# Neuroprosthetics-Lab/nejm-brain-to-text

Hardware: AMD Instinct MI355X
Metric: GRU+CTC train sentences/sec (higher is better)
Workload: dtype f32; 1 GPU; BASELINE.json configs[1]: 5-layer GRU-512 + CTC, synthetic [B=64,T=500,F=512] -> 41 phonemes, fp32, full training step incl. on-GPU augmentation, clip and AdamW; global_batch=64, rows_per_rank=64, seq_len=500, parallelism=dp1, world_size_seen=1, gru_mode=1

## Files before the change

nejm-brain-to-text_amd/csrc/gemm.hip:

```cpp
#include "common.h"
#include "gemm_args.h"

namespace b2t {

using f32x16 = float __attribute__((ext_vector_type(16)));
using f32x4 = float __attribute__((ext_vector_type(4)));

#ifndef B2T_GEMM_BK
#define B2T_GEMM_BK 16
#endif
#ifndef B2T_GEMM_OCC
#define B2T_GEMM_OCC 3
#endif
constexpr int BM = 128, BN = 128, BKT = B2T_GEMM_BK;
constexpr int NLD = BKT / 8;
constexpr int TPR = BKT / 4;
constexpr int RPP = 256 / TPR;
template <bool KC> struct Pitch { static constexpr int v = KC ? 129 : 132; };
constexpr int PITCH_MAX = 132;

template <bool KC>
__device__ __forceinline__ void load_full(const float* __restrict__ P, const long long (&roff)[NLD], int mcl, int k0,
                                          long long s0, long long s1, int div, float4 (&v)[NLD], int tid) {
#pragma unroll
  for (int r = 0; r < NLD; ++r) {
    if constexpr (KC) {
      v[r] = *reinterpret_cast<const float4*>(P + roff[r] + k0 + (tid % TPR) * 4);
    } else {
      v[r] = *reinterpret_cast<const float4*>(P + rowoff(k0 + (tid >> 5) + 8 * r, s0, s1, div) + mcl);
    }
  }
}

template <bool KC>
__device__ __forceinline__ void load_tail(const float* __restrict__ P, const long long (&roff)[NLD], int ext_m,
                                          int base_m, int k0, int Kend, long long s0, long long s1, int div,
                                          float4 (&v)[NLD], int tid) {
#pragma unroll
  for (int r = 0; r < NLD; ++r) {
    float4 o = make_float4(0.f, 0.f, 0.f, 0.f);
    if constexpr (KC) {
      const int row = base_m + tid / TPR + RPP * r;
      const int k = k0 + (tid % TPR) * 4;
      if (row < ext_m) {
        const float* p = P + roff[r] + k;
        if (k < Kend) o.x = p[0];
        if (k + 1 < Kend) o.y = p[1];
        if (k + 2 < Kend) o.z = p[2];
        if (k + 3 < Kend) o.w = p[3];
      }
    } else {
      const int k = k0 + (tid >> 5) + 8 * r;
      const int m = base_m + (tid & 31) * 4;
      if (k < Kend) {
        const float* p = P + rowoff(k, s0, s1, div) + m;
        if (m < ext_m) o.x = p[0];
        if (m + 1 < ext_m) o.y = p[1];
        if (m + 2 < ext_m) o.z = p[2];
        if (m + 3 < ext_m) o.w = p[3];
      }
    }
    v[r] = o;
  }
}

template <bool KC>
__device__ __forceinline__ void store_tile(float* __restrict__ S, const float4 (&v)[NLD], int tid) {
  constexpr int PITCH = Pitch<KC>::v;
#pragma unroll
  for (int r = 0; r < NLD; ++r) {
    if constexpr (KC) {
      const int row = tid / TPR + RPP * r;
      const int k = (tid % TPR) * 4;
      S[(k + 0) * PITCH + row] = v[r].x;
      S[(k + 1) * PITCH + row] = v[r].y;
      S[(k + 2) * PITCH + row] = v[r].z;
      S[(k + 3) * PITCH + row] = v[r].w;
    } else {
      const int k = (tid >> 5) + 8 * r;
      const int m = (tid & 31) * 4;
      *reinterpret_cast<float4*>(&S[k * PITCH + m]) = v[r];
    }
  }
}

__device__ __forceinline__ float4 load_f4_sc1(const float* base_uniform, unsigned byte_off) {
  using u32x4 = unsigned int __attribute__((ext_vector_type(4)));
  __amdgpu_buffer_rsrc_t rsrc = __builtin_amdgcn_make_buffer_rsrc(const_cast<float*>(base_uniform), 0, 0x7fffffff, 0x00020000);
  const u32x4 v = __builtin_amdgcn_raw_buffer_load_b128(rsrc, byte_off, 0, 16);
  return make_float4(__uint_as_float(v.x), __uint_as_float(v.y), __uint_as_float(v.z), __uint_as_float(v.w));
}

template <bool AKC, bool BKC>
__global__ __launch_bounds__(256, B2T_GEMM_OCC) void gemm_f32_kernel(GemmArgs g) {
  __shared__ __attribute__((aligned(16))) float smem[2 * 2 * BKT * PITCH_MAX];
  constexpr int PA = Pitch<AKC>::v, PB = Pitch<BKC>::v;
  float* As = smem;
  float* Bs = smem + 2 * BKT * PITCH_MAX;

  const int tid = threadIdx.x;
  const int lane = tid & 63, wave = tid >> 6;
  const int wm = wave >> 1, wn = wave & 1;
  int z = blockIdx.z / g.splitk;
  int ks = blockIdx.z - z * g.splitk;
  int m0, n0;
  {
    const int gx = (g.N + BN - 1) / BN, nwg = gridDim.x;
    int tile;
    if (g.ks_xcd) {
      const int lin = blockIdx.x + nwg * blockIdx.z, xcd = lin & 7, j = lin >> 3;
      ks = xcd + 8 * (j / nwg); tile = j % nwg; z = 0;
    } else {
      const int b = blockIdx.x, xcd = b & 7, qq = nwg >> 3, rr = nwg & 7;
      tile = (xcd < rr ? xcd * (qq + 1) : rr * (qq + 1) + (xcd - rr) * qq) + (b >> 3);
    }
    m0 = (tile / gx) * BM; n0 = (tile % gx) * BN;
  }

  const float* A = g.A + (long long)z * g.a_sz;
  const int zb = g.b_zmap ? g.b_zmap[z] : z;
  const float* B = g.B + (long long)zb * g.b_sz;
  const float* bias = (g.bias && ks == 0) ? g.bias + (long long)zb * g.bias_sz : nullptr;
  float* C = g.C + (long long)z * g.c_sz + (long long)ks * g.c_ks;

  long long roffA[NLD], roffB[NLD];
#pragma unroll
  for (int r = 0; r < NLD; ++r) {
    const int ra_ = m0 + tid / TPR + RPP * r, rb_ = n0 + tid / TPR + RPP * r;
    roffA[r] = AKC ? rowoff(ra_ < g.M ? ra_ : g.M - 1, g.a_s0, g.a_s1, g.a_div) : 0;
    roffB[r] = BKC ? rowoff(rb_ < g.N ? rb_ : g.N - 1, g.b_s0, g.b_s1, g.b_div) : 0;
  }
  const int mclA = min(m0 + (tid & 31) * 4, ((g.M + 3) & ~3) - 4);
  const int mclB = min(n0 + (tid & 31) * 4, ((g.N + 3) & ~3) - 4);

  f32x16 acc[2][2];
#pragma unroll
  for (int i = 0; i < 2; ++i)
#pragma unroll
    for (int j = 0; j < 2; ++j)
#pragma unroll
      for (int e = 0; e < 16; ++e) acc[i][j][e] = 0.f;

  const int kb = ks * g.kchunk;
  const int K = min(g.K, kb + g.kchunk);
  const int nk = (K - kb + BKT - 1) / BKT;
  const int nfull = (K - kb) / BKT;
  float4 ra[NLD], rb[NLD];

  auto fetch = [&](int kt) {
    const int k0 = kb + kt * BKT;
    const float* Ag = A + ((g.a_brk > 0 && (AKC ? k0 : m0) >= g.a_brk) ? g.a_gap : 0);
    if (kt < nfull) {
      load_full<AKC>(Ag, roffA, mclA, k0, g.a_s0, g.a_s1, g.a_div, ra, tid);
      load_full<BKC>(B, roffB, mclB, k0, g.b_s0, g.b_s1, g.b_div, rb, tid);
    } else {
      load_tail<AKC>(Ag, roffA, g.M, m0, k0, K, g.a_s0, g.a_s1, g.a_div, ra, tid);
      load_tail<BKC>(B, roffB, g.N, n0, k0, K, g.b_s0, g.b_s1, g.b_div, rb, tid);
    }
  };
  const bool do_sum = !AKC && g.a_sum != nullptr && n0 == 0;
  float4 asum = make_float4(0.f, 0.f, 0.f, 0.f);
  auto add_a = [&]() {
    if constexpr (!AKC) {
      if (do_sum) {
#pragma unroll
        for (int r = 0; r < NLD; ++r) { asum.x += ra[r].x; asum.y += ra[r].y; asum.z += ra[r].z; asum.w += ra[r].w; }
      }
    }
  };
  fetch(0);
  add_a();
  store_tile<AKC>(As, ra, tid);
  store_tile<BKC>(Bs, rb, tid);
  __syncthreads();

  const int lk = lane >> 5, li = lane & 31;
  int cur = 0;
  for (int kt = 0; kt < nk; ++kt) {
    const bool more = kt + 1 < nk;
    if (more) fetch(kt + 1);
    const float* as = As + cur * BKT * PA + wm * 64 + li + lk * PA;
    const float* bs = Bs + cur * BKT * PB + wn * 64 + li + lk * PB;
    float a0 = as[0], a1 = as[32], b0 = bs[0], b1 = bs[32];
#pragma unroll
    for (int kk = 0; kk < BKT; kk += 2) {
      float na0 = 0.f, na1 = 0.f, nb0 = 0.f, nb1 = 0.f;
      if (kk + 2 < BKT) {
        na0 = as[(kk + 2) * PA]; na1 = as[(kk + 2) * PA + 32];
        nb0 = bs[(kk + 2) * PB]; nb1 = bs[(kk + 2) * PB + 32];
      }
      acc[0][0] = __builtin_amdgcn_mfma_f32_32x32x2f32(a0, b0, acc[0][0], 0, 0, 0);
      acc[0][1] = __builtin_amdgcn_mfma_f32_32x32x2f32(a0, b1, acc[0][1], 0, 0, 0);
      acc[1][0] = __builtin_amdgcn_mfma_f32_32x32x2f32(a1, b0, acc[1][0], 0, 0, 0);
      acc[1][1] = __builtin_amdgcn_mfma_f32_32x32x2f32(a1, b1, acc[1][1], 0, 0, 0);
      a0 = na0; a1 = na1; b0 = nb0; b1 = nb1;
    }
    if (more) {
      add_a();
      store_tile<AKC>(As + (cur ^ 1) * BKT * PA, ra, tid);
      store_tile<BKC>(Bs + (cur ^ 1) * BKT * PB, rb, tid);
    }
    __syncthreads();
    cur ^= 1;
  }

  if constexpr (!AKC) {
    if (do_sum) {
      float4* red = reinterpret_cast<float4*>(smem);
      red[tid] = asum;
      __syncthreads();
      if (tid < 32) {
        float4 t = red[tid];
#pragma unroll
        for (int gq = 1; gq < 8; ++gq) { const float4 u = red[gq * 32 + tid]; t.x += u.x; t.y += u.y; t.z += u.z; t.w += u.w; }
        float* o = g.a_sum + ((long long)z * g.splitk + ks) * g.a_sum_ks;
        const int m = m0 + tid * 4;
        if (m < g.M) o[m] = t.x;
        if (m + 1 < g.M) o[m + 1] = t.y;
        if (m + 2 < g.M) o[m + 2] = t.z;
        if (m + 3 < g.M) o[m + 3] = t.w;
      }
    }
  }
#pragma unroll
  for (int i = 0; i < 2; ++i) {
#pragma unroll
    for (int j = 0; j < 2; ++j) {
      const int col = n0 + wn * 64 + j * 32 + li;
      if (col >= g.N) continue;
      const float bv = bias ? bias[col] : 0.f;
#pragma unroll
      for (int e = 0; e < 16; ++e) {
        const int row = m0 + wm * 64 + i * 32 + (e & 3) + 8 * (e >> 2) + 4 * lk;
        if (row < g.M) {
          float v = acc[i][j][e] + bv;
          if (g.epilogue == 1) v = v / (1.0f + fabsf(v));
          const long long coff = rowoff(row, g.c_s0, g.c_s1, g.c_div) + col;
          if (g.epilogue == 2) { const float a = 1.0f - fabsf(g.ep_aux[(long long)z * g.c_sz + coff]); v *= a * a; }
          float* p = C + coff;
          if (g.accumulate) v += *p;
          if (g.ks_cnt) __hip_atomic_store(p, v, __ATOMIC_RELAXED, __HIP_MEMORY_SCOPE_AGENT);
          else *p = v;
        }
      }
    }
  }
  if (g.ks_cnt) {
    asm volatile("s_waitcnt vmcnt(0)" ::: "memory");
    __syncthreads();
    int* flag = reinterpret_cast<int*>(smem);
    const int gx = (g.N + BN - 1) / BN, tile_id = (m0 / BM) * gx + n0 / BN;
    if (tid == 0) {
      const unsigned old = __hip_atomic_fetch_add(g.ks_cnt + tile_id, 1u, __ATOMIC_RELAXED, __HIP_MEMORY_SCOPE_AGENT);
      const int last = old == (unsigned)g.splitk - 1u;
      if (last) __hip_atomic_store(g.ks_cnt + tile_id, 0u, __ATOMIC_RELAXED, __HIP_MEMORY_SCOPE_AGENT);
      flag[0] = last;
    }
    __syncthreads();
    if (flag[0]) {
      for (int idx = tid; idx < BM * (BN / 4); idx += 256) {
        const int r = m0 + idx / (BN / 4), cc = n0 + (idx % (BN / 4)) * 4;
        if (r >= g.M || cc >= g.N) continue;
        const long long e = (long long)r * g.N + cc;
        float4 acc = make_float4(0.f, 0.f, 0.f, 0.f);
        if (g.ks_acc) acc = *reinterpret_cast<const float4*>(g.ks_out + e);
        for (int sl = 0; sl < g.splitk; ++sl) {
          const float4 v = load_f4_sc1(g.C + (long long)sl * g.c_ks, (unsigned)(e * 4));
          acc.x += v.x; acc.y += v.y; acc.z += v.z; acc.w += v.w;
        }
        *reinterpret_cast<float4*>(g.ks_out + e) = acc;
      }
    }
  }
}


template <int MT, bool BKC>
__global__ __launch_bounds__(512) void gemm_skinny_kernel(GemmArgs g) {
  __shared__ float red[8][MT][4][64];
  const int tid = threadIdx.x, lane = tid & 63, wave = tid >> 6;
  const int j = lane & 15, q = lane >> 4;
  const int n0 = blockIdx.x * 16;
  const int z = blockIdx.y, zb = g.b_zmap ? g.b_zmap[z] : z;
  g.A += (long long)z * g.a_sz; g.B += (long long)zb * g.b_sz; g.C += (long long)z * g.c_sz;
  if (g.bias) g.bias += (long long)zb * g.bias_sz;
  const int ncol = n0 + j < g.N ? n0 + j : g.N - 1;
  const float* brow = BKC ? g.B + rowoff(ncol, g.b_s0, g.b_s1, g.b_div) + 4 * q : g.B + ncol;
  const float* arow[MT];
#pragma unroll
  for (int mt = 0; mt < MT; ++mt) {
    const int r = 16 * mt + j;
    arow[mt] = g.A + rowoff(r < g.M ? r : g.M - 1, g.a_s0, g.a_s1, g.a_div) + 4 * q;
  }
  f32x4 acc[MT];
#pragma unroll
  for (int mt = 0; mt < MT; ++mt) acc[mt] = f32x4{0.f, 0.f, 0.f, 0.f};
  const int nchunk = g.K / 16;
  for (int c0 = wave * 4; c0 < nchunk; c0 += 32) {
    float4 bw[4], av[4][MT];
#pragma unroll
    for (int u = 0; u < 4; ++u) {
      const int k = (c0 + u < nchunk ? c0 + u : c0) * 16;
      if constexpr (BKC) {
        bw[u] = *reinterpret_cast<const float4*>(brow + k);
      } else {
        const int kq = k + 4 * q;
        bw[u] = make_float4(brow[rowoff(kq, g.b_s0, g.b_s1, g.b_div)], brow[rowoff(kq + 1, g.b_s0, g.b_s1, g.b_div)],
                            brow[rowoff(kq + 2, g.b_s0, g.b_s1, g.b_div)], brow[rowoff(kq + 3, g.b_s0, g.b_s1, g.b_div)]);
      }
#pragma unroll
      for (int mt = 0; mt < MT; ++mt) av[u][mt] = *reinterpret_cast<const float4*>(arow[mt] + k);
    }
#pragma unroll
    for (int u = 0; u < 4; ++u) {
      if (c0 + u < nchunk) {
#pragma unroll
        for (int mt = 0; mt < MT; ++mt) {
          acc[mt] = __builtin_amdgcn_mfma_f32_16x16x4f32(av[u][mt].x, bw[u].x, acc[mt], 0, 0, 0);
          acc[mt] = __builtin_amdgcn_mfma_f32_16x16x4f32(av[u][mt].y, bw[u].y, acc[mt], 0, 0, 0);
          acc[mt] = __builtin_amdgcn_mfma_f32_16x16x4f32(av[u][mt].z, bw[u].z, acc[mt], 0, 0, 0);
          acc[mt] = __builtin_amdgcn_mfma_f32_16x16x4f32(av[u][mt].w, bw[u].w, acc[mt], 0, 0, 0);
        }
      }
    }
  }
#pragma unroll
  for (int mt = 0; mt < MT; ++mt)
#pragma unroll
    for (int e = 0; e < 4; ++e) red[wave][mt][e][lane] = acc[mt][e];
  __syncthreads();
  for (int idx = tid; idx < MT * 4 * 64; idx += 512) {
    const int l = idx & 63, e = (idx >> 6) & 3, mt = idx >> 8;
    const float v0 = (red[0][mt][e][l] + red[1][mt][e][l]) + (red[2][mt][e][l] + red[3][mt][e][l]);
    const float v1 = (red[4][mt][e][l] + red[5][mt][e][l]) + (red[6][mt][e][l] + red[7][mt][e][l]);
    const int row = 16 * mt + 4 * (l >> 4) + e, col = n0 + (l & 15);
    if (row < g.M && col < g.N) {
      float v = v0 + v1 + (g.bias ? g.bias[col] : 0.f);
      if (g.epilogue == 1) v = v / (1.0f + fabsf(v));
      float* p = g.C + rowoff(row, g.c_s0, g.c_s1, g.c_div) + col;
      if (g.accumulate) v += *p;
      *p = v;
    }
  }
}

}

extern "C" int b2t_gemm_f32(const b2t_gemm_desc* d, void* stream) {
  using namespace b2t;
  B2T_REQUIRE(d != nullptr, "b2t_gemm_f32: null descriptor");
  B2T_REQUIRE(d->M > 0 && d->N > 0 && d->K > 0 && d->Z > 0, "b2t_gemm_f32: bad shape M=%d N=%d K=%d Z=%d",
              d->M, d->N, d->K, d->Z);
  B2T_REQUIRE(((uintptr_t)d->A & 15) == 0 && ((uintptr_t)d->B & 15) == 0, "b2t_gemm_f32: A/B must be 16-byte aligned");
  B2T_REQUIRE((d->a_s0 % 4) == 0 && (d->a_s1 % 4) == 0 && (d->a_sz % 4) == 0 && (d->b_s0 % 4) == 0 &&
                  (d->b_s1 % 4) == 0 && (d->b_sz % 4) == 0,
              "b2t_gemm_f32: A/B strides must be multiples of 4 elements");
  B2T_REQUIRE(d->a_sum == nullptr || !d->a_kcontig, "b2t_gemm_f32: a_sum goes with an m-contiguous A (a_kcontig = 0)");
  B2T_REQUIRE(d->ks_counters == nullptr || (d->splitk > 1 && d->Z == 1 && (d->N % 4) == 0 && d->ks_out != nullptr && ((uintptr_t)d->ks_out & 15) == 0 &&
                                            (long long)d->M * d->N * 4 < (1ll << 31)),
              "b2t_gemm_f32: the in-kernel slab reduction needs splitk > 1, Z = 1, N %% 4 == 0 and a 16-byte aligned ks_out");
  GemmArgs g;
  { int rc = fill_gemm_args(d, g, BKT, BM, "b2t_gemm_f32"); if (rc) return rc; }
  dim3 grid(((d->N + BN - 1) / BN) * ((d->M + BM - 1) / BM), 1, d->Z * g.splitk), block(256);
  { static const bool off = getenv("B2T_GEMM_KS_XCD") && atoi(getenv("B2T_GEMM_KS_XCD")) == 0; g.ks_xcd = !off && d->Z == 1 && g.splitk >= 8 && (g.splitk & 7) == 0; }
  hipStream_t s = as_stream(stream);
  if (d->M <= 64 && d->splitk >= 0 && g.splitk == 1 && d->a_kcontig && (d->K % 16) == 0 && d->a_brk == 0 && d->epilogue != 2) {
    const dim3 sg((d->N + 15) / 16, d->Z), sb(512);
#define B2T_SKINNY(MT)                                                                                  \
    do {                                                                                                \
      if (d->b_kcontig) hipLaunchKernelGGL((gemm_skinny_kernel<MT, true>), sg, sb, 0, s, g);              \
      else hipLaunchKernelGGL((gemm_skinny_kernel<MT, false>), sg, sb, 0, s, g);                          \
    } while (0)
    if (d->M <= 16) B2T_SKINNY(1);
    else if (d->M <= 32) B2T_SKINNY(2);
    else if (d->M <= 48) B2T_SKINNY(3);
    else B2T_SKINNY(4);
#undef B2T_SKINNY
    B2T_CHECK_LAUNCH("b2t_gemm_f32 (skinny)");
    return 0;
  }
  if (d->a_kcontig && d->b_kcontig) hipLaunchKernelGGL((gemm_f32_kernel<true, true>), grid, block, 0, s, g);
  else if (d->a_kcontig && !d->b_kcontig) hipLaunchKernelGGL((gemm_f32_kernel<true, false>), grid, block, 0, s, g);
  else if (!d->a_kcontig && d->b_kcontig) hipLaunchKernelGGL((gemm_f32_kernel<false, true>), grid, block, 0, s, g);
  else hipLaunchKernelGGL((gemm_f32_kernel<false, false>), grid, block, 0, s, g);
  B2T_CHECK_LAUNCH("b2t_gemm_f32");
  return 0;
}
```

Baseline: 3437 sentences/s.

## Use incremental address cursors and split main/tail loops in f32 GEMM

Replaces per-iteration rowoff index arithmetic with pointer cursors that advance by precomputed uniform strides, handling the div wrap and gap with selects. The k-loop is split into a steady full-tile loop without tail branching, separated by sched barriers, and a peeled tail. Launch bounds rise to occupancy 4 and the compile-time BK/OCC knobs are removed. This aims to cut VALU address work and register pressure in the GEMM main loop, at the cost of extra complexity and a possible correctness risk in the cursor wrap logic.

```diff
diff --git a/nejm-brain-to-text_amd/csrc/gemm.hip b/nejm-brain-to-text_amd/csrc/gemm.hip
--- a/nejm-brain-to-text_amd/csrc/gemm.hip
+++ b/nejm-brain-to-text_amd/csrc/gemm.hip
@@ -6,44 +6,84 @@
 using f32x16 = float __attribute__((ext_vector_type(16)));
 using f32x4 = float __attribute__((ext_vector_type(4)));
 
-#ifndef B2T_GEMM_BK
-#define B2T_GEMM_BK 16
-#endif
-#ifndef B2T_GEMM_OCC
-#define B2T_GEMM_OCC 3
-#endif
-constexpr int BM = 128, BN = 128, BKT = B2T_GEMM_BK;
+constexpr int BM = 128, BN = 128, BKT = 16;
 constexpr int NLD = BKT / 8;
 constexpr int TPR = BKT / 4;
 constexpr int RPP = 256 / TPR;
 template <bool KC> struct Pitch { static constexpr int v = KC ? 129 : 132; };
 constexpr int PITCH_MAX = 132;
 
+template <bool KC> struct Cursor {
+  const float* p[NLD];
+  int rem[NLD];
+  long long d0, d1;
+  int dv, stepr;
+};
+
+__device__ __forceinline__ int uniform(int v) { return __builtin_amdgcn_readfirstlane(v); }
+__device__ __forceinline__ long long uniform(long long v) {
+  return (long long)(((unsigned long long)(unsigned)uniform((int)(v >> 32)) << 32) | (unsigned)uniform((int)v));
+}
+
 template <bool KC>
-__device__ __forceinline__ void load_full(const float* __restrict__ P, const long long (&roff)[NLD], int mcl, int k0,
-                                          long long s0, long long s1, int div, float4 (&v)[NLD], int tid) {
+__device__ __forceinline__ void cursor_init(Cursor<KC>& c, const float* __restrict__ P, int base, int ext, int kb,
+                                            long long s0, long long s1, int div, int tid) {
+  if constexpr (KC) {
+#pragma unroll
+    for (int r = 0; r < NLD; ++r) {
+      const int row = base + tid / TPR + RPP * r;
+      c.p[r] = P + rowoff(row < ext ? row : ext - 1, s0, s1, div) + kb + (tid % TPR) * 4;
+      c.rem[r] = 0;
+    }
+    c.d0 = BKT; c.d1 = 0; c.dv = 0; c.stepr = 0;
+  } else {
+    c.dv = uniform(div > 0 ? div : 0x7fffffff);
+    c.stepr = uniform(BKT % c.dv);
+    c.d0 = uniform((long long)(BKT / c.dv) * s1 + (long long)c.stepr * s0);
+    c.d1 = uniform(s1 - (long long)c.dv * s0);
+    const int mcl = min(base + (tid & 31) * 4, ((ext + 3) & ~3) - 4);
+#pragma unroll
+    for (int r = 0; r < NLD; ++r) {
+      const int k = kb + (tid >> 5) + 8 * r;
+      c.rem[r] = k % c.dv;
+      c.p[r] = P + (long long)(k / c.dv) * s1 + (long long)c.rem[r] * s0 + mcl;
+    }
+  }
+}
+
+template <bool KC>
+__device__ __forceinline__ void cursor_next(Cursor<KC>& c, long long extra) {
 #pragma unroll
   for (int r = 0; r < NLD; ++r) {
     if constexpr (KC) {
-      v[r] = *reinterpret_cast<const float4*>(P + roff[r] + k0 + (tid % TPR) * 4);
+      c.p[r] += BKT + extra;
     } else {
-      v[r] = *reinterpret_cast<const float4*>(P + rowoff(k0 + (tid >> 5) + 8 * r, s0, s1, div) + mcl);
+      const int over = c.rem[r] + (c.stepr - c.dv);
+      const bool wrap = over >= 0;
+      c.rem[r] = wrap ? over : over + c.dv;
+      const float* same = c.p[r] + c.d0;
+      const float* wrapped = c.p[r] + (c.d0 + c.d1);
+      c.p[r] = wrap ? wrapped : same;
     }
   }
 }
 
 template <bool KC>
-__device__ __forceinline__ void load_tail(const float* __restrict__ P, const long long (&roff)[NLD], int ext_m,
-                                          int base_m, int k0, int Kend, long long s0, long long s1, int div,
-                                          float4 (&v)[NLD], int tid) {
+__device__ __forceinline__ void load_full(const Cursor<KC>& c, float4 (&v)[NLD]) {
+#pragma unroll
+  for (int r = 0; r < NLD; ++r) v[r] = *reinterpret_cast<const float4*>(c.p[r]);
+}
+
+template <bool KC>
+__device__ __forceinline__ void load_tail(const Cursor<KC>& c, int ext_m, int base_m, int k0, int Kend, float4 (&v)[NLD], int tid) {
 #pragma unroll
   for (int r = 0; r < NLD; ++r) {
     float4 o = make_float4(0.f, 0.f, 0.f, 0.f);
+    const float* p = c.p[r];
     if constexpr (KC) {
       const int row = base_m + tid / TPR + RPP * r;
       const int k = k0 + (tid % TPR) * 4;
       if (row < ext_m) {
-        const float* p = P + roff[r] + k;
         if (k < Kend) o.x = p[0];
         if (k + 1 < Kend) o.y = p[1];
         if (k + 2 < Kend) o.z = p[2];
@@ -53,7 +93,6 @@
       const int k = k0 + (tid >> 5) + 8 * r;
       const int m = base_m + (tid & 31) * 4;
       if (k < Kend) {
-        const float* p = P + rowoff(k, s0, s1, div) + m;
         if (m < ext_m) o.x = p[0];
         if (m + 1 < ext_m) o.y = p[1];
         if (m + 2 < ext_m) o.z = p[2];
@@ -84,6 +123,24 @@
   }
 }
 
+template <int PA, int PB>
+__device__ __forceinline__ void mma_tile(const float* __restrict__ as, const float* __restrict__ bs, f32x16 (&acc)[2][2]) {
+  float a0 = as[0], a1 = as[32], b0 = bs[0], b1 = bs[32];
+#pragma unroll
+  for (int kk = 0; kk < BKT; kk += 2) {
+    float na0 = 0.f, na1 = 0.f, nb0 = 0.f, nb1 = 0.f;
+    if (kk + 2 < BKT) {
+      na0 = as[(kk + 2) * PA]; na1 = as[(kk + 2) * PA + 32];
+      nb0 = bs[(kk + 2) * PB]; nb1 = bs[(kk + 2) * PB + 32];
+    }
+    acc[0][0] = __builtin_amdgcn_mfma_f32_32x32x2f32(a0, b0, acc[0][0], 0, 0, 0);
+    acc[0][1] = __builtin_amdgcn_mfma_f32_32x32x2f32(a0, b1, acc[0][1], 0, 0, 0);
+    acc[1][0] = __builtin_amdgcn_mfma_f32_32x32x2f32(a1, b0, acc[1][0], 0, 0, 0);
+    acc[1][1] = __builtin_amdgcn_mfma_f32_32x32x2f32(a1, b1, acc[1][1], 0, 0, 0);
+    a0 = na0; a1 = na1; b0 = nb0; b1 = nb1;
+  }
+}
+
 __device__ __forceinline__ float4 load_f4_sc1(const float* base_uniform, unsigned byte_off) {
   using u32x4 = unsigned int __attribute__((ext_vector_type(4)));
   __amdgpu_buffer_rsrc_t rsrc = __builtin_amdgcn_make_buffer_rsrc(const_cast<float*>(base_uniform), 0, 0x7fffffff, 0x00020000);
@@ -92,7 +149,7 @@
 }
 
 template <bool AKC, bool BKC>
-__global__ __launch_bounds__(256, B2T_GEMM_OCC) void gemm_f32_kernel(GemmArgs g) {
+__global__ __launch_bounds__(256, 4) void gemm_f32_kernel(GemmArgs g) {
   __shared__ __attribute__((aligned(16))) float smem[2 * 2 * BKT * PITCH_MAX];
   constexpr int PA = Pitch<AKC>::v, PB = Pitch<BKC>::v;
   float* As = smem;
@@ -123,16 +180,6 @@
   const float* bias = (g.bias && ks == 0) ? g.bias + (long long)zb * g.bias_sz : nullptr;
   float* C = g.C + (long long)z * g.c_sz + (long long)ks * g.c_ks;
 
-  long long roffA[NLD], roffB[NLD];
-#pragma unroll
-  for (int r = 0; r < NLD; ++r) {
-    const int ra_ = m0 + tid / TPR + RPP * r, rb_ = n0 + tid / TPR + RPP * r;
-    roffA[r] = AKC ? rowoff(ra_ < g.M ? ra_ : g.M - 1, g.a_s0, g.a_s1, g.a_div) : 0;
-    roffB[r] = BKC ? rowoff(rb_ < g.N ? rb_ : g.N - 1, g.b_s0, g.b_s1, g.b_div) : 0;
-  }
-  const int mclA = min(m0 + (tid & 31) * 4, ((g.M + 3) & ~3) - 4);
-  const int mclB = min(n0 + (tid & 31) * 4, ((g.N + 3) & ~3) - 4);
-
   f32x16 acc[2][2];
 #pragma unroll
   for (int i = 0; i < 2; ++i)
@@ -144,20 +191,16 @@
   const int kb = ks * g.kchunk;
   const int K = min(g.K, kb + g.kchunk);
   const int nk = (K - kb + BKT - 1) / BKT;
-  const int nfull = (K - kb) / BKT;
+  const int nfull = uniform(K > kb ? (K - kb) / BKT : 0);
+
+  const bool gap0 = g.a_brk > 0 && (AKC ? kb : m0) >= g.a_brk;
+  const int kgap = (AKC && g.a_brk > kb) ? g.a_brk : -1;
+  Cursor<AKC> ca;
+  Cursor<BKC> cb;
+  cursor_init<AKC>(ca, A + (gap0 ? g.a_gap : 0), m0, g.M, kb, g.a_s0, g.a_s1, g.a_div, tid);
+  cursor_init<BKC>(cb, B, n0, g.N, kb, g.b_s0, g.b_s1, g.b_div, tid);
   float4 ra[NLD], rb[NLD];
 
-  auto fetch = [&](int kt) {
-    const int k0 = kb + kt * BKT;
-    const float* Ag = A + ((g.a_brk > 0 && (AKC ? k0 : m0) >= g.a_brk) ? g.a_gap : 0);
-    if (kt < nfull) {
-      load_full<AKC>(Ag, roffA, mclA, k0, g.a_s0, g.a_s1, g.a_div, ra, tid);
-      load_full<BKC>(B, roffB, mclB, k0, g.b_s0, g.b_s1, g.b_div, rb, tid);
-    } else {
-      load_tail<AKC>(Ag, roffA, g.M, m0, k0, K, g.a_s0, g.a_s1, g.a_div, ra, tid);
-      load_tail<BKC>(B, roffB, g.N, n0, k0, K, g.b_s0, g.b_s1, g.b_div, rb, tid);
-    }
-  };
   const bool do_sum = !AKC && g.a_sum != nullptr && n0 == 0;
   float4 asum = make_float4(0.f, 0.f, 0.f, 0.f);
   auto add_a = [&]() {
@@ -168,53 +211,70 @@
       }
     }
   };
-  fetch(0);
+  auto next = [&](int k0) {
+    cursor_next<AKC>(ca, AKC && k0 == kgap ? g.a_gap : 0);
+    cursor_next<BKC>(cb, 0);
+  };
+  if (nfull > 0) {
+    load_full<AKC>(ca, ra);
+    load_full<BKC>(cb, rb);
+    next(kb + BKT);
+  } else {
+    load_tail<AKC>(ca, g.M, m0, kb, K, ra, tid);
+    load_tail<BKC>(cb, g.N, n0, kb, K, rb, tid);
+  }
   add_a();
   store_tile<AKC>(As, ra, tid);
   store_tile<BKC>(Bs, rb, tid);
   __syncthreads();
 
   const int lk = lane >> 5, li = lane & 31;
+  const float* as = As + wm * 64 + li + lk * PA;
+  const float* bs = Bs + wn * 64 + li + lk * PB;
   int cur = 0;
-  for (int kt = 0; kt < nk; ++kt) {
-    const bool more = kt + 1 < nk;
-    if (more) fetch(kt + 1);
-    const float* as = As + cur * BKT * PA + wm * 64 + li + lk * PA;
-    const float* bs = Bs + cur * BKT * PB + wn * 64 + li + lk * PB;
-    float a0 = as[0], a1 = as[32], b0 = bs[0], b1 = bs[32];
-#pragma unroll
-    for (int kk = 0; kk < BKT; kk += 2) {
-      float na0 = 0.f, na1 = 0.f, nb0 = 0.f, nb1 = 0.f;
-      if (kk + 2 < BKT) {
-        na0 = as[(kk + 2) * PA]; na1 = as[(kk + 2) * PA + 32];
-        nb0 = bs[(kk + 2) * PB]; nb1 = bs[(kk + 2) * PB + 32];
-      }
-      acc[0][0] = __builtin_amdgcn_mfma_f32_32x32x2f32(a0, b0, acc[0][0], 0, 0, 0);
-      acc[0][1] = __builtin_amdgcn_mfma_f32_32x32x2f32(a0, b1, acc[0][1], 0, 0, 0);
-      acc[1][0] = __builtin_amdgcn_mfma_f32_32x32x2f32(a1, b0, acc[1][0], 0, 0, 0);
-      acc[1][1] = __builtin_amdgcn_mfma_f32_32x32x2f32(a1, b1, acc[1][1], 0, 0, 0);
-      a0 = na0; a1 = na1; b0 = nb0; b1 = nb1;
-    }
-    if (more) {
-      add_a();
-      store_tile<AKC>(As + (cur ^ 1) * BKT * PA, ra, tid);
-      store_tile<BKC>(Bs + (cur ^ 1) * BKT * PB, rb, tid);
-    }
+#pragma unroll 1
+  for (int kt = 1; kt < nfull; ++kt) {
+    load_full<AKC>(ca, ra);
+    load_full<BKC>(cb, rb);
+    next(kb + (kt + 1) * BKT);
+    __builtin_amdgcn_sched_barrier(0);
+    mma_tile<PA, PB>(as + cur * BKT * PA, bs + cur * BKT * PB, acc);
+    __builtin_amdgcn_sched_barrier(0);
+    cur ^= 1;
+    add_a();
+    store_tile<AKC>(As + cur * BKT * PA, ra, tid);
+    store_tile<BKC>(Bs + cur * BKT * PB, rb, tid);
     __syncthreads();
+  }
+  int tp = tid;
+  asm volatile("" : "+v"(tp));
+  const bool tail = nfull > 0 && nk > nfull;
+  if (tail) {
+    load_tail<AKC>(ca, g.M, m0, kb + nfull * BKT, K, ra, tp);
+    load_tail<BKC>(cb, g.N, n0, kb + nfull * BKT, K, rb, tp);
+  }
+  if (nk > 0) mma_tile<PA, PB>(as + cur * BKT * PA, bs + cur * BKT * PB, acc);
+  if (tail) {
     cur ^= 1;
+    add_a();
+    store_tile<AKC>(As + cur * BKT * PA, ra, tp);
+    store_tile<BKC>(Bs + cur * BKT * PB, rb, tp);
+    __syncthreads();
+    mma_tile<PA, PB>(as + cur * BKT * PA, bs + cur * BKT * PB, acc);
   }
 
   if constexpr (!AKC) {
     if (do_sum) {
+      __syncthreads();
       float4* red = reinterpret_cast<float4*>(smem);
-      red[tid] = asum;
+      red[tp] = asum;
       __syncthreads();
-      if (tid < 32) {
-        float4 t = red[tid];
-#pragma unroll
-        for (int gq = 1; gq < 8; ++gq) { const float4 u = red[gq * 32 + tid]; t.x += u.x; t.y += u.y; t.z += u.z; t.w += u.w; }
+      if (tp < 32) {
+        float4 t = red[tp];
+#pragma unroll
+        for (int gq = 1; gq < 8; ++gq) { const float4 u = red[gq * 32 + tp]; t.x += u.x; t.y += u.y; t.z += u.z; t.w += u.w; }
         float* o = g.a_sum + ((long long)z * g.splitk + ks) * g.a_sum_ks;
-        const int m = m0 + tid * 4;
+        const int m = m0 + tp * 4;
         if (m < g.M) o[m] = t.x;
         if (m + 1 < g.M) o[m + 1] = t.y;
         if (m + 2 < g.M) o[m + 2] = t.z;
@@ -222,16 +282,17 @@
       }
     }
   }
+  const int li2 = tp & 31, lk2 = (tp & 63) >> 5, wm2 = tp >> 7, wn2 = (tp >> 6) & 1;
 #pragma unroll
   for (int i = 0; i < 2; ++i) {
 #pragma unroll
     for (int j = 0; j < 2; ++j) {
-      const int col = n0 + wn * 64 + j * 32 + li;
+      const int col = n0 + wn2 * 64 + j * 32 + li2;
       if (col >= g.N) continue;
       const float bv = bias ? bias[col] : 0.f;
 #pragma unroll
       for (int e = 0; e < 16; ++e) {
-        const int row = m0 + wm * 64 + i * 32 + (e & 3) + 8 * (e >> 2) + 4 * lk;
+        const int row = m0 + wm2 * 64 + i * 32 + (e & 3) + 8 * (e >> 2) + 4 * lk2;
         if (row < g.M) {
           float v = acc[i][j][e] + bv;
           if (g.epilogue == 1) v = v / (1.0f + fabsf(v));
```

Result: no change. 3444 sentences/s, median of 5 (+0.2%).
